# patrickzbhe/ray-tracing-series-rust

Hardware: AMD Instinct MI355X
Metric: Msamples/s (pixels x spp) on Book-1 final scene (higher is better)
Workload: dtype f64

## Files before the change

ray-tracing-series-rust_amd/csrc/hip/render.hip:

```cpp
#include <hip/hip_runtime.h>
#include <cstdio>
#include <cstdlib>
#include <algorithm>
#include <chrono>
#include <cfloat>
#include <cmath>
#include <cstring>
#include <new>
#include <type_traits>
#include <utility>
#include <string>
#include <vector>
#include "../../../include/rtx_abi.h"
#include "../core/cull32.hpp"
#include "../core/integrator.hpp"
#include "../core/occlusion.hpp"
#include "../core/item_order.hpp"
#include "../core/karras.hpp"
#include "../core/mover_box.hpp"
#include "../core/prim_box.hpp"
#include "../host/flat_scene.hpp"
#include "../host/light_table.hpp"
#include "../host/update_shadow.hpp"
#include "../host/set_shading.hpp"
#include "../host/wide_tree.hpp"
#include "device_buffer.hpp"
#include "f32_bridge.hpp"
#ifndef RTX_F32_TU
#include "abi_internal.hpp"
#include "../host/set_triangles.hpp"
#else
namespace rtx { void set_error(const std::string& msg); }
#endif

namespace rtx {

#include "lds_layout.inc"
#include "lds_variant.inc"
static_assert(LDSV_TIME_BOXES == RTX_LDS_VARIANT_TIME_BOXES && LDSV_ONE_AXIS == RTX_LDS_VARIANT_ONE_AXIS &&
              LDSV_COMMON_RATIO == RTX_LDS_VARIANT_COMMON_RATIO, "RtxRenderStats.trace_variant");
#include "pass_items.inc"

typedef const FlatNode4 FlatNode4Dev;
struct WorldDesc;

struct VoteTop {
  int32_t n;
  int32_t all_rects;
  int32_t k[8];
  uint32_t ref[8];
  rt::FlatRect rect[8];
};

enum class ForcedKernel { none, simple, vote, world, wavefront };

struct TraceSwitches {
  ForcedKernel kernel = ForcedKernel::none;
  bool diag = false;
  int ring = -1, wide = -1, scene_lds = -1;
  bool vote_top = true, tri_direct = true, mat_lds = true, perlin_lds = true;
  bool mv_common = true, motion = true, motion_axis = true;
  bool single_leaf = true, pass_pipeline = true, validate = false;
  uint32_t chunk = TRACE_CHUNK;
  uint32_t item_group = 0;
  uint32_t world_threshold = 8;
  uint32_t walk_threshold = 0, regen_min = 0, leaf_weight = 0;
  uint32_t wf_paths = 1u << 22, wf_refill = 16, wf_check = 8;
  int wf_occ = 4;
  bool wf_verbose = false;
};

struct Workspace {
  DeviceBuffer<double> samples;
  DeviceBuffer<double> accum;
  DeviceBuffer<rt::TraceCounters> counters;
  DeviceBuffer<unsigned int> work_counter;
  DeviceBuffer<PassMap> pass_map;
  DeviceBuffer<unsigned long long> diag;
  hipEvent_t ev[2] = {nullptr, nullptr};
  hipStream_t aux_stream = nullptr;
  hipEvent_t ev_pass[3] = {nullptr, nullptr, nullptr};
  DeviceBuffer<unsigned char> wave_mem;
  uint32_t* wave_host_ctrl = nullptr;
};

struct VotePlan {
  bool ok = false;
  int32_t bvh_pos = 0;
  int32_t tri_base = -1;
  VoteTop top;
  int blocks_per_cu[2] = {1, 1};
  bool ring[2] = {false, false};
  uint32_t tables = 0;
  size_t tables_bytes = 0;
};

struct WidePlan {
  FlatNode4Dev* nodes4 = nullptr;
  int levels = 0;
  int vote_blocks_per_cu = 1;
};

struct WorldPlan {
  const WorldDesc* desc = nullptr;
  uint32_t mat_lds = 0, tex_lds = 0;
  uint32_t perlin_lds = 0;
  int blocks_per_cu[5][2] = {{1, 1}, {1, 1}, {1, 1}, {1, 1}, {1, 1}};
};

struct LdsFit {
  bool ok = false;
  uint32_t ring_cap = 0;
  uint32_t levels = 0;
  LdsSceneDims dims = {0, 0, 0, 0, 0, 0};
};

struct LdsPlan {
  LdsFit plain;
  LdsFit motion;
  int motion_axis = -1;
  double motion_t0 = 0.0, motion_t1 = 0.0;
  bool motion_planned = false;
  uint32_t lds_max = 0;
  bool mv_common = false;
  double mv_t0 = 0.0, mv_t1 = 1.0;
};

struct WalkTuning {
  uint32_t walk_threshold = 18;
  uint32_t regen_min = 1;
  uint32_t leaf_weight = 3;
  bool single_leaf = false;
  uint32_t item_group_lds = 2, item_group_vote = rt::ITEM_GROUP_MAX, item_group_world = 4,
           item_group_wavefront = rt::ITEM_GROUP_MAX, item_group_simple = rt::ITEM_GROUP_MAX;
};

struct SceneUpdate {
  UpdateShadow shadow;
  std::vector<double> local_box;
  size_t n_entries = 0, n_nodes = 0, n_motion = 0, n_desc = 0;
  size_t n_triangles = 0, n_top = 0, n_spheres = 0, n_moving_spheres = 0, n_rects = 0;
  DeviceBuffer<double> d_local_box;
  DeviceBuffer<int32_t> d_leaf_parent, d_node_parent;
  DeviceBuffer<unsigned int> d_arrivals;
  DeviceBuffer<rt::XformOp64> d_slot_ops64;
  StagingBuffer staging;
  ShadingShadow shading;
  int32_t member_stack = 0;
  std::vector<int32_t> tree_depth;
  size_t n_perlins = 0, n_materials = 0, n_textures = 0;
  DeviceBuffer<double> r_boxes, r_bounds, r_box64, r_terms;
  DeviceBuffer<unsigned long long> r_keys, r_keys_sorted;
  DeviceBuffer<uint32_t> r_vals, r_vals_sorted;
  DeviceBuffer<int32_t> r_children, r_parent_node, r_parent_leaf, r_leaf_parent, r_node_parent, r_depth;
  DeviceBuffer<rt::FlatNode> r_nodes;
  DeviceBuffer<rt::FlatNode32> r_nodes32;
  DeviceBuffer<rt::FlatMotion32> r_motion32;
  DeviceBuffer<unsigned char> r_sort_temp;
};

#ifndef RTX_F32_TU
struct MeshUpdate {
  MeshShadow shadow;
  bool uploaded = false;
  DeviceBuffer<int32_t> d_leaves, d_node_parent;
  DeviceBuffer<unsigned int> d_arrivals;
  StagingBuffer staging;
  bool local_box_stale = false;
  std::vector<char> sphere_is_light;
  std::vector<char> rect_is_light;
  DeviceBuffer<double> d_light_weight;
  std::vector<unsigned int> slope_mask;
  DeviceBuffer<unsigned int> d_slope_mask;
  DeviceBuffer<double> d_end_boxes;
  ReadbackWords slope_readback;
};
#endif

struct DeviceScene {
  int device = -1;
  std::vector<DeviceBuffer<void>> allocations;
  rt::SceneView view;
  size_t scene_bytes = 0;
  int n_cu = 256;
  double gravity_time_limit = 1e300;
  TraceSwitches sw;
  Workspace ws;
  VotePlan vote;
  WidePlan wide;
  WorldPlan world;
  LdsPlan lds;
  WalkTuning walk;
  rt::LightView lights = {nullptr, nullptr, 0, 0};
  SceneUpdate upd;
#ifndef RTX_F32_TU
  MeshUpdate mesh;
#endif
};

#define HIP_TRY(expr)                                                                      \
  do {                                                                                     \
    hipError_t _e = (expr);                                                                \
    if (_e != hipSuccess) {                                                                \
      set_error(std::string(#expr) + ": " + hipGetErrorString(_e));                        \
      return RTX_EHIP;                                                                     \
    }                                                                                      \
  } while (0)

template <class T>
static rtx_status upload_array(DeviceScene* ds, const std::vector<T>& v, const T** out) {
  *out = nullptr;
  if (v.empty()) return RTX_OK;
  DeviceBuffer<void> b;
  size_t bytes = v.size() * sizeof(T);
  HIP_TRY(b.alloc(bytes));
// ... 61 lines not shown
#include "trace_vote.inc"
#include "trace_world.inc"
#include "trace_lds.inc"
#include "trace_wave.inc"
#include "post_kernels.inc"
#include "denoise.inc"
#include "cast_rays.inc"
#include "trace_rays.inc"
#include "occlusion.inc"
#ifndef RTX_F32_TU
#include "trace_nee.inc"
#endif
#include "scene_update.inc"
static size_t stack_bytes(uint32_t levels);
static void plan_world_stacks(DeviceScene* ds);
#include "scene_rebuild.inc"
#ifndef RTX_F32_TU
#include "mesh_update.inc"
#endif
#include "shading_update.inc"
#include "cull_hooks.inc"

static int shard_row_count(int32_t height, const RtxShard& sh, int32_t row_limit) {
  int n = 0;
  for (int32_t j = 0; j < height && j < row_limit; ++j)
    if ((j / sh.block_rows) % sh.shard_count == sh.shard_index) ++n;
  return n;
}

static rtx_status validate(const void* s, const RtxCamera* cam, const RtxConfig* cfg,
                           const RtxShard* shard, RtxShard* sh_out) {
  if (!s || !cam || !cfg) { set_error("render: NULL scene, camera or config"); return RTX_EINVAL; }
  if (cfg->threads <= 0 || cfg->image_width <= 0 || cfg->samples_per_pixel <= 0 || cfg->max_depth <= 0) {
    set_error("render: Config::new asserts threads, image_width, samples_per_pixel, max_depth > 0 (world.rs:36-40)");
    return RTX_EINVAL;
  }
  if (rtx_image_height(cfg) <= 0) { set_error("render: image height <= 0 (Screen::new asserts, screen.rs:14)"); return RTX_EINVAL; }
  if (!(cam->time1 < cam->time2)) { set_error("render: camera time1 >= time2 (gen_range panics on an empty range, camera.rs:69)"); return RTX_EINVAL; }
  RtxShard sh = {0, 1, 1, 0};
  if (shard) sh = *shard;
  if (sh.shard_count <= 0 || sh.shard_index < 0 || sh.shard_index >= sh.shard_count || sh.block_rows <= 0) {
    set_error("render: bad shard");
    return RTX_EINVAL;
  }
  *sh_out = sh;
  return RTX_OK;
}

static rt::RenderParams make_params(const RtxCamera* cam, const RtxConfig* cfg) {
  rt::RenderParams rp;
  static_assert(sizeof(RtxCamera) == 24 * sizeof(double) && sizeof(rt::FlatCamera) == 24 * sizeof(rt::real), "camera layout");
  for (int k = 0; k < 24; ++k) ((rt::real*)&rp.cam)[k] = (rt::real)((const double*)cam)[k];
  rp.background = rt::v3(cfg->background[0], cfg->background[1], cfg->background[2]);
  rp.image_width = cfg->image_width;
  rp.image_height = rtx_image_height(cfg);
  rp.samples_per_pixel = cfg->samples_per_pixel;
  rp.max_depth = cfg->max_depth;
  rp.seed = cfg->seed;
  return rp;
}

static TraceSwitches read_switches() {
  auto num = [](const char* n, int lo, int hi, uint32_t dflt) { const char* s = getenv(n); return s && atoi(s) >= lo && atoi(s) <= hi ? (uint32_t)atoi(s) : dflt; };
  auto flag = [](const char* n) { const char* s = getenv(n); return s ? (atoi(s) != 0 ? 1 : 0) : -1; };
  TraceSwitches sw;
  if (const char* k = getenv("RTX_TRACE_KERNEL")) {
    const std::string s = k;
    if (s == "simple") sw.kernel = ForcedKernel::simple;
    else if (s == "vote" || s == "vote_diag") sw.kernel = ForcedKernel::vote;
    else if (s == "world" || s == "world_diag") sw.kernel = ForcedKernel::world;
    else if (s == "wavefront") sw.kernel = ForcedKernel::wavefront;
    sw.diag = s == "vote_diag" || s == "world_diag";
  }
  sw.ring = flag("RTX_RING"); sw.wide = flag("RTX_WIDE"); sw.scene_lds = flag("RTX_SCENE_LDS");
  sw.vote_top = flag("RTX_VOTE_TOP") != 0; sw.tri_direct = flag("RTX_TRI_DIRECT") != 0;
  sw.mat_lds = flag("RTX_MAT_LDS") != 0; sw.perlin_lds = flag("RTX_PERLIN_LDS") != 0;
  sw.mv_common = flag("RTX_MV_COMMON") != 0; sw.motion = flag("RTX_MOTION") != 0; sw.motion_axis = flag("RTX_MOTION_AXIS") != 0;
  sw.single_leaf = flag("RTX_SINGLE_LEAF") != 0; sw.pass_pipeline = flag("RTX_PASS_PIPELINE") != 0;
  sw.validate = getenv("RTX_VALIDATE") != nullptr;
  sw.chunk = num("RTX_CHUNK", 64, 65536, sw.chunk);
  sw.item_group = num("RTX_ITEM_GROUP", 1, (int)rt::ITEM_GROUP_MAX, 0);
  sw.world_threshold = num("RTX_WORLD_THRESHOLD", 0, 64, sw.world_threshold);
  sw.walk_threshold = num("RTX_WALK_THRESHOLD", 1, 64, 0); sw.regen_min = num("RTX_REGEN_MIN", 1, 64, 0); sw.leaf_weight = num("RTX_LEAF_WEIGHT", 1, 64, 0);
  const char* wp = getenv("RTX_WF_PATHS");
  if (wp && atol(wp) >= 256 && atol(wp) <= (1l << 27)) sw.wf_paths = (uint32_t)atol(wp);
  sw.wf_refill = num("RTX_WF_REFILL", 1, 64, sw.wf_refill); sw.wf_check = num("RTX_WF_CHECK", 1, 4096, sw.wf_check);
  sw.wf_occ = (int)num("RTX_WF_OCC", 4, 6, (uint32_t)sw.wf_occ); sw.wf_verbose = getenv("RTX_WF_VERBOSE") != nullptr;
  return sw;
}

static size_t stack_bytes(uint32_t levels) { return (size_t)levels * TRACE_BLOCK * sizeof(int32_t); }

template <class K>
static int occupancy(K kernel, size_t lds) {
  int nb = 0;
  return hipOccupancyMaxActiveBlocksPerMultiprocessor(&nb, kernel, TRACE_BLOCK, lds) == hipSuccess ? nb : 0;
}

static uint32_t grid_size(uint32_t total, uint32_t block, uint64_t resident) {
  const uint64_t want = ((uint64_t)total + block - 1) / block;
  return (uint32_t)(want < resident ? want : resident);
}

struct PassArgs {
  rt::RenderParams rp;
  ShardMap sm;
  uint32_t s_begin, total, npix;
  double* samples;
  unsigned int* work_counter;
  hipStream_t stream;
  int preset;
  uint32_t feat;
  uint32_t stack_levels;
  size_t stack_lds;
  const uint32_t* active;
};

template <class Launch>
static void with_map(const PassArgs& a, Launch launch) {
  if (a.active) launch(ActiveMap{a.sm, a.active});
  else launch(a.sm);
}

template <class Launch>
static rtx_status run_diag(DeviceScene* ds, hipStream_t stream, Launch launch, const char* tag, int width, const char* const* names,
                           int n, unsigned long long (&h)[24]) {
  if (!ds->ws.diag) HIP_TRY(ds->ws.diag.alloc(sizeof(h)));
  HIP_TRY(hipMemsetAsync(ds->ws.diag, 0, sizeof(h), stream));
  launch();
  HIP_TRY(hipStreamSynchronize(stream));
  HIP_TRY(hipMemcpy(h, ds->ws.diag, sizeof(h), hipMemcpyDeviceToHost));
  for (int k = 0; k < n; ++k)
    fprintf(stderr, "[%s] %-*s executions %llu lanes %llu mean lanes %.2f\n", tag, width, names[k], h[2 * k], h[2 * k + 1],
            h[2 * k] ? (double)h[2 * k + 1] / (double)h[2 * k] : 0.0);
  return RTX_OK;
}

struct LeafScan { uint32_t max_count = 0, max_end = 0; };
static LeafScan scan_leaves(const FlatScene& fs) {
  LeafScan s;
  for (const rt::FlatNode& nd : fs.nodes)
    for (int ch = 0; ch < 2; ++ch)
      if (nd.child[ch] < 0) {
        s.max_count = std::max(s.max_count, rt::leaf_count(nd.child[ch]));
        s.max_end = std::max(s.max_end, rt::leaf_first(nd.child[ch]) + rt::leaf_count(nd.child[ch]));
      }
  return s;
}

static void plan_vote(DeviceScene* ds, const FlatScene& fs) {
  VotePlan& p = ds->vote;
  const TraceSwitches& sw = ds->sw;
  const size_t lds = stack_bytes((uint32_t)fs.max_stack + 1u), lds_ring = lds + (TRACE_BLOCK / 64) * ring_bytes(64);
  const bool ring_fits = lds_ring <= 64 * 1024;
  auto fit = [&](int preset, int nb0, int nb1, bool ring_by_default) {
    p.ring[preset] = ring_by_default && nb1 > 0 && nb1 >= nb0 && ring_fits;
    if (sw.ring >= 0 && nb1 > 0 && ring_fits) p.ring[preset] = sw.ring != 0;
    const int nb = p.ring[preset] ? nb1 : nb0;
    if (nb > 0) p.blocks_per_cu[preset] = nb;
  };
  fit(0, occupancy(k_trace_vote<P_SPHERES, false, false, false>, lds), occupancy(k_trace_vote<P_SPHERES, false, true, false>, lds_ring), true);
  fit(1, occupancy(k_trace_vote<P_MESH, false, false, false>, lds), occupancy(k_trace_vote<P_MESH, false, true, false>, lds_ring), false);

  memset(&p.top, 0, sizeof(p.top));
  p.top.n = -1;
  int n_bvh = 0, n_other = 0;
// ... 242 lines not shown
static void plan_lds_motion_axis(LdsPlan* p, const TraceSwitches& sw, uint32_t slope_mask) {
  const bool y_only = slope_mask == 2u && sw.motion_axis;
  p->motion_axis = y_only ? 1 : -1;
  p->motion.dims.node_dwords = y_only ? LDSK_MOTION1_NODE_DWORDS : LDSK_MOTION_NODE_DWORDS;
  p->motion.ok = false;
  p->motion.ring_cap = 0;
  if (p->motion_planned && p->plain.ok) fit_lds(&p->motion, sw.ring != 0, p->lds_max);
}

static rtx_status plan_lds(DeviceScene* ds, const FlatScene& fs, const LeafScan& leaves) {
  const bool single_bvh = fs.top_level.size() == 1 && fs.entries[fs.top_level[0]].kind == rt::ENTRY_BVH;
  if (!single_bvh || (fs.features & ~P_SPHERES) != 0 || fs.nodes32.size() > LDSK_MAX_NODES) return RTX_OK;
  LdsPlan& p = ds->lds;
  const TraceSwitches& sw = ds->sw;
  const uint32_t max_end = leaves.max_end, levels = (uint32_t)fs.max_stack + 1u;
  int lds_max = 0;
  (void)hipDeviceGetAttribute(&lds_max, hipDeviceAttributeMaxSharedMemoryPerBlock, ds->device);
  if (lds_max > (int)LDSK_LDS_MAX) lds_max = (int)LDSK_LDS_MAX;
  p.plain.levels = levels;
  p.plain.dims = {(uint32_t)fs.nodes32.size(), max_end, max_end, 0u, LDSK_NODE_DWORDS, 0u};
  p.mv_common = sw.mv_common && lds_common_interval(fs.moving_spheres.data(), fs.moving_spheres.size(), &p.mv_t0, &p.mv_t1);
  uint32_t counts[3];
  lds_record_counts(fs.features, P_STATIC_SPHERES, (uint32_t)fs.spheres.size(), max_end, counts);
  p.plain.dims.n_spheres = counts[0]; p.plain.dims.n_moving = counts[1]; p.plain.dims.n_uni = counts[2];
  p.motion.levels = levels;
  p.motion.dims = p.plain.dims;
  p.motion.dims.node_dwords = LDSK_MOTION_NODE_DWORDS;
  if (leaves.max_count <= 4 && max_end <= LDSK_MAX_SLOTS && sw.scene_lds != 0 && lds_max > 0) {
    const bool want_ring = sw.ring != 0;
    fit_lds(&p.plain, want_ring, (uint32_t)lds_max);
    const rt::FlatEntry& be = fs.entries[fs.top_level[0]];
    if (p.plain.ok && !fs.motion32.empty() && (fs.features & rt::F_MOVING_SPHERE) && lds_motion_interval_ok((double)be.f[0], (double)be.f[1]) && sw.motion) {
      p.motion_t0 = (double)be.f[0]; p.motion_t1 = (double)be.f[1];
      p.motion_planned = true;
      p.lds_max = (uint32_t)lds_max;
    }
  }
  plan_lds_motion_axis(&p, sw, rt::motion_slope_mask(fs.motion32.data(), fs.motion32.size()));
  if (p.plain.ok) {
    hipError_t ae = hipSuccess;
    bool static_lds = false;
    hipFuncAttributes fa;
#define LDS_ATTR1(K)                                                                                                   \
  if (ae == hipSuccess) ae = hipFuncSetAttribute((const void*)K, hipFuncAttributeMaxDynamicSharedMemorySize, lds_max); \
  if (ae == hipSuccess) ae = hipFuncGetAttributes(&fa, (const void*)K);                                                \
  if (ae == hipSuccess && fa.sharedSizeBytes != 0) static_lds = true
#define LDS_ATTR(FEAT, RINGF, MOTIONF) LDS_ATTR1((k_trace_lds<FEAT, RINGF, MOTIONF>)); LDS_ATTR1((k_trace_lds<FEAT, RINGF, MOTIONF, ActiveMap>))
    LDS_ATTR(P_SPHERES, true, 0u); LDS_ATTR(P_SPHERES, false, 0u); LDS_ATTR(P_STATIC_SPHERES, true, 0u); LDS_ATTR(P_STATIC_SPHERES, false, 0u);
    LDS_ATTR(P_SPHERES, true, 1u); LDS_ATTR(P_SPHERES, false, 1u); LDS_ATTR(P_SPHERES, true, 3u); LDS_ATTR(P_SPHERES, false, 3u);
#undef LDS_ATTR
#undef LDS_ATTR1
    if (ae != hipSuccess) { (void)hipGetLastError(); p.plain.ok = false; p.motion.ok = false; }
    if (static_lds) {
      fprintf(stderr, "[rtx] k_trace_lds has static LDS in front of its node array: not used\n");
      p.plain.ok = false; p.motion.ok = false;
    }
  }
  if (sw.scene_lds >= 0) {
    auto bytes = [](const LdsFit& f) { return f.ok ? ldsk_layout(f.levels, f.ring_cap, f.dims).total : 0u; };
    fprintf(stderr, "[rtx] RTX_SCENE_LDS: k_trace_lds %s (ring of %u, %u B of LDS); time-aware boxes %s (ring of %u, %u B)\n",
            p.plain.ok ? "on" : "off", p.plain.ring_cap, ldsk_layout(levels, p.plain.ring_cap, p.plain.dims).total,
            p.motion.ok ? "on" : "off", p.motion.ring_cap, bytes(p.motion));
  }
  return RTX_OK;
}

static rtx_status launch_lds(DeviceScene* ds, const PassArgs& a, const RtxCamera* cam, int32_t* variant) {
#ifndef RTX_F32_TU
  if (ds->mesh.slope_readback.pending()) {
    const unsigned int* words = nullptr;
    HIP_TRY(ds->mesh.slope_readback.wait(&words));
    plan_lds_motion_axis(&ds->lds, ds->sw, words[0]);
  }
#endif
  const LdsPlan& p = ds->lds;
  *variant = lds_trace_variant(p.motion.ok, p.motion_t0, p.motion_t1, (double)cam->time1, (double)cam->time2, p.motion_axis, p.mv_common);
  const bool motion = (*variant & LDSV_TIME_BOXES) != 0;
  const LdsFit& f = motion ? p.motion : p.plain;
  const bool ring = f.ring_cap != 0u;
  const rt::real m_t0 = (rt::real)p.motion_t0, m_inv = (rt::real)(1.0 / (p.motion_t1 - p.motion_t0));
  const LdsKernelLayout L = ldsk_layout(f.levels, f.ring_cap, f.dims);
  const uint32_t grid = grid_size(a.total, LDSK_BLOCK, (uint64_t)ds->n_cu);
  const WalkTuning& wk = ds->walk;
#define LAUNCH_LDS2(FEAT, RINGF, MOTIONF)                                                                               \
  with_map(a, [&](auto map) {                                                                                           \
    hipLaunchKernelGGL(HIP_KERNEL_NAME(k_trace_lds<FEAT, RINGF, MOTIONF, decltype(map)>), dim3(grid), dim3(LDSK_BLOCK), L.total, \
                       a.stream, ds->view, a.rp, map, a.s_begin, a.total, a.samples, a.work_counter, wk.leaf_weight, \
                       wk.walk_threshold | (wk.single_leaf ? 0x100u : 0u), ds->sw.chunk, f.ring_cap, f.levels, f.dims,  \
                       m_t0, m_inv, p.mv_common ? 1u : 0u, (rt::real)p.mv_t0, (rt::real)p.mv_t1);                        \
  })
#define LAUNCH_LDS(FEAT, MOTIONF) do { if (ring) { LAUNCH_LDS2(FEAT, true, MOTIONF); } else { LAUNCH_LDS2(FEAT, false, MOTIONF); } } while (0)
  if (!lds_records_are_moving(a.feat, P_STATIC_SPHERES)) { LAUNCH_LDS(P_STATIC_SPHERES, 0u); }
  else if (*variant & LDSV_ONE_AXIS) { LAUNCH_LDS(P_SPHERES, 3u); }
  else if (motion) { LAUNCH_LDS(P_SPHERES, 1u); }
  else { LAUNCH_LDS(P_SPHERES, 0u); }
#undef LAUNCH_LDS
#undef LAUNCH_LDS2
  return RTX_OK;
}

template <bool COUNT>
static void launch_simple(const DeviceScene* ds, const PassArgs& a) {
  const uint32_t grid = grid_size(a.total, TRACE_BLOCK, (uint64_t)ds->n_cu * 8);
#define LAUNCH_SIMPLE2(FEAT, MAP)                                                                                       \
  hipLaunchKernelGGL(HIP_KERNEL_NAME(k_trace_simple<FEAT, COUNT, decltype(MAP)>), dim3(grid), dim3(TRACE_BLOCK), a.stack_lds, \
                     a.stream, ds->view, a.rp, MAP, a.s_begin, a.total, a.samples, ds->ws.counters)
#define LAUNCH_SIMPLE(FEAT) with_map(a, [&](auto map) { LAUNCH_SIMPLE2(FEAT, map); })
  const bool inst = (a.feat & rt::F_INSTANCE) != 0;
  if constexpr (COUNT) {
    if (inst) { LAUNCH_SIMPLE2(P_INST, a.sm); } else { LAUNCH_SIMPLE2(P_ALL, a.sm); }
  } else {
    if (a.preset == 0) { LAUNCH_SIMPLE(P_SPHERES); }
    else if (a.preset == 1) { LAUNCH_SIMPLE(P_MESH); }
    else if (inst) { LAUNCH_SIMPLE(P_INST); }
    else { LAUNCH_SIMPLE(P_ALL); }
  }
#undef LAUNCH_SIMPLE
#undef LAUNCH_SIMPLE2
}

#ifndef RTX_F32_TU
static rtx_status launch_nee(const DeviceScene* ds, const PassArgs& a) {
  const int preset = (a.feat & rt::F_INSTANCE) ? 3 : ((a.feat & ~P_MESH_ROOM) == 0 ? 0 : ((a.feat & rt::F_GRAVITY_SPHERE) ? 2 : 1));
#define LAUNCH_NEE(FEAT, MAP)                                                                                                   \
  do {                                                                                                                          \
    const int nb = occupancy(k_trace_nee<FEAT, decltype(MAP)>, a.stack_lds);                                                    \
    const uint32_t grid = grid_size(a.total, TRACE_CHUNK, (uint64_t)ds->n_cu * (uint64_t)(nb > 0 ? nb : 1) * (TRACE_BLOCK / 64)); \
    hipLaunchKernelGGL(HIP_KERNEL_NAME(k_trace_nee<FEAT, decltype(MAP)>), dim3((grid + TRACE_BLOCK / 64 - 1) / (TRACE_BLOCK / 64)),     \
                       dim3(TRACE_BLOCK), a.stack_lds, a.stream, ds->view, ds->lights, a.rp, MAP, a.s_begin, a.total,     \
                       a.samples, a.work_counter);                                                                              \
  } while (0)
  with_map(a, [&](auto map) {
    if (preset == 0) LAUNCH_NEE(P_MESH_ROOM, map);
    else if (preset == 1) LAUNCH_NEE(P_ANY, map);
    else if (preset == 3) LAUNCH_NEE(P_INST, map);
    else LAUNCH_NEE(P_ALL, map);
  });
#undef LAUNCH_NEE
  return RTX_OK;
}
#endif

static rtx_status wave_pass(DeviceScene* ds, const PassArgs& a) {
  Workspace& ws = ds->ws;
  const hipStream_t stream = a.stream;
  uint32_t P = ds->sw.wf_paths;
  if ((uint64_t)P > (uint64_t)a.total) P = a.total;
  P = (P + WF_SEG - 1u) & ~(WF_SEG - 1u);
  const uint32_t n_seg = P / WF_SEG;
  const size_t R = sizeof(rt::real);
  const size_t bytes = 64 + (size_t)P * (16 + 7 * R + 3 * R + 3 * R + R + 4 + 4 + 4 + 4) + (size_t)n_seg * 8;
  HIP_TRY(ws.wave_mem.grow(bytes, stream));
  if (!ws.wave_host_ctrl) HIP_TRY(hipHostMalloc((void**)&ws.wave_host_ctrl, 4 * sizeof(uint32_t), hipHostMallocDefault));
  WavePool pool;
  {
    unsigned char* m = ws.wave_mem;
    pool.ctrl = (uint32_t*)m; m += 64;
    pool.rng = (unsigned long long*)m; m += (size_t)P * 16;
    pool.ray = (rt::real*)m; m += (size_t)P * 7 * R;
    pool.product = (rt::real*)m; m += (size_t)P * 3 * R;
    pool.output = (rt::real*)m; m += (size_t)P * 3 * R;
    pool.hit_t = (rt::real*)m; m += (size_t)P * R;
    pool.depth = (int32_t*)m; m += (size_t)P * 4;
    pool.g = (uint32_t*)m; m += (size_t)P * 4;
    pool.hit_ref = (uint32_t*)m; m += (size_t)P * 4;
    pool.free_list = (uint32_t*)m; m += (size_t)P * 4;
    pool.n_free = (uint32_t*)m; m += (size_t)n_seg * 4;
    pool.cursor = (uint32_t*)m; m += (size_t)n_seg * 4;
    pool.P = P;
  }
  const int preset = a.preset;
  const bool wide = preset == 1 && ds->wide.nodes4 != nullptr;
  const uint32_t levels = wide ? (uint32_t)ds->wide.levels : a.stack_levels;
  const size_t lds = stack_bytes(levels);
  if (lds > 64 * 1024) { set_error("render: BVH too deep for the LDS traversal stack"); return RTX_EUNSUPPORTED; }
  const bool room = (a.feat & ~P_MESH_ROOM) == 0;
  const int occ = ds->sw.wf_occ;
  const uint32_t leaf_weight = ds->walk.leaf_weight, refill = ds->sw.wf_refill, bvh_pos = (uint32_t)ds->vote.bvh_pos;
#define WF_CASES(X)                                                                                                          \
  if (preset == 0) { X(P_SPHERES, false, 4); }                                                                               \
  else if (!wide) { X(P_MESH, false, 4); }                                                                                   \
  else if (room && occ == 5) { X(P_MESH_ROOM, true, 5); }                                                                    \
  else if (room && occ == 6) { X(P_MESH_ROOM, true, 6); }                                                                    \
  else if (room) { X(P_MESH_ROOM, true, 4); }                                                                                \
  else { X(P_MESH, true, 4); }
  int nb = 0;
  hipError_t oe = hipSuccess;
#define WF_OCC(FEAT, WIDEF, MB) oe = hipOccupancyMaxActiveBlocksPerMultiprocessor(&nb, k_wf_trace<FEAT, WIDEF, MB>, TRACE_BLOCK, lds)
  WF_CASES(WF_OCC)
#undef WF_OCC
  if (oe != hipSuccess || nb <= 0) { (void)hipGetLastError(); nb = 1; }
  const uint32_t tgrid = grid_size(P, TRACE_BLOCK, (uint64_t)ds->n_cu * (uint64_t)nb);
  hipLaunchKernelGGL(k_wf_init, dim3((P + 255u) / 256u), dim3(256), 0, stream, pool);
  uint32_t check_every = ds->sw.wf_check;
  int it = 0;
  for (;; ++it) {
    with_map(a, [&](auto map) {
      hipLaunchKernelGGL(HIP_KERNEL_NAME(k_wf_generate<decltype(map)>), dim3(n_seg), dim3(WF_SEG), 0, stream, pool, a.rp, map,
                         a.s_begin, a.total);
    });
    if ((uint32_t)(it + 1) % check_every == 0u) {
      HIP_TRY(hipMemsetAsync(pool.ctrl, 0, 16, stream));
      hipLaunchKernelGGL(k_wf_count, dim3(256), dim3(256), 0, stream, pool);
      HIP_TRY(hipGetLastError());
      HIP_TRY(hipMemcpyAsync(ws.wave_host_ctrl, pool.ctrl, 4 * sizeof(uint32_t), hipMemcpyDeviceToHost, stream));
      HIP_TRY(hipStreamSynchronize(stream));
      if (ws.wave_host_ctrl[0] == 0u) break;
      if (ws.wave_host_ctrl[0] < P / 2u) check_every = 2;
      if (it > 100000000) { set_error("render: wavefront integrator did not converge"); return RTX_EHIP; }
    }
#define WF_LAUNCH(FEAT, WIDEF, MB)                                                                                           \
  do {                                                                                                                       \
    hipLaunchKernelGGL(HIP_KERNEL_NAME(k_wf_trace<FEAT, WIDEF, MB>), dim3(tgrid), dim3(TRACE_BLOCK), lds, stream, ds->view, pool, \
                       leaf_weight, refill, bvh_pos, ds->wide.nodes4, ds->vote.tri_base);                                    \
    hipLaunchKernelGGL(HIP_KERNEL_NAME(k_wf_shade<FEAT>), dim3(n_seg), dim3(WF_SEG), 0, stream, ds->view, pool, a.rp, a.samples, bvh_pos); \
  } while (0)
    WF_CASES(WF_LAUNCH)
#undef WF_LAUNCH
  }
#undef WF_CASES
  if (ds->sw.wf_verbose) fprintf(stderr, "[rtx] wavefront: %u slots, %d iterations, %d blocks per CU (%u stack levels)\n", P, it + 1, nb, levels);
  return RTX_OK;
}

static void plan_walk(DeviceScene* ds, const LeafScan& leaves) {
  WalkTuning& w = ds->walk;
  const TraceSwitches& sw = ds->sw;
  w.leaf_weight = leaves.max_count <= 1 ? 1u : 3u;
  w.single_leaf = leaves.max_count <= 1;
  if (ds->wide.nodes4) { w.leaf_weight = 1u; w.walk_threshold = 24u; w.regen_min = 8u; }
  else if (ds->lds.plain.ok) w.walk_threshold = 12u;
  if (sw.regen_min) w.regen_min = sw.regen_min;
  if (sw.leaf_weight) w.leaf_weight = sw.leaf_weight;
  if (!sw.single_leaf) w.single_leaf = false;
  if (sw.walk_threshold) w.walk_threshold = sw.walk_threshold;
  if (sw.item_group) w.item_group_lds = w.item_group_vote = w.item_group_world = w.item_group_wavefront = w.item_group_simple = sw.item_group;
}

static uint32_t item_group_of(const WalkTuning& w, int32_t kernel) {
  switch (kernel) {
    case RTX_KERNEL_SIMPLE: return w.item_group_simple;
    case RTX_KERNEL_LDS: return w.item_group_lds;
    case RTX_KERNEL_WAVEFRONT: return w.item_group_wavefront;
    case RTX_KERNEL_VOTE: return w.item_group_vote;
    default: return w.item_group_world;
  }
}

static int32_t choose_trace_kernel(const DeviceScene* ds, int preset, bool count) {
  const ForcedKernel k = ds->sw.kernel;
  if (count || k == ForcedKernel::simple) return RTX_KERNEL_SIMPLE;
  if (ds->lds.plain.ok && preset == 0 && k == ForcedKernel::none) return RTX_KERNEL_LDS;
  if (ds->vote.ok && preset < 2 && k == ForcedKernel::wavefront) return RTX_KERNEL_WAVEFRONT;
  if (ds->vote.ok && preset < 2 && k != ForcedKernel::world) return RTX_KERNEL_VOTE;
  return RTX_KERNEL_WORLD;
}

typedef RtxSampleRange SampleRange;

struct PassPlan {
  uint32_t spp_pass;
  bool pipeline;
  size_t sample_bytes;
};

static rtx_status prepare_workspace(DeviceScene* ds, uint64_t sample_buffer_bytes, uint64_t npix, uint64_t npix_all, uint32_t spp,
                                    bool serial, hipStream_t stream, double** accum, PassPlan* pp) {
  Workspace& ws = ds->ws;
  uint64_t budget = sample_buffer_bytes;
  if (budget == 0) {
    budget = 24ull << 30;
    size_t free_b = 0, total_b = 0;
    if (hipMemGetInfo(&free_b, &total_b) == hipSuccess) {
      const uint64_t avail = ((uint64_t)free_b + ws.samples.bytes()) / 3;
      if (avail < budget) budget = avail;
    } else {
      (void)hipGetLastError();
    }
    if (budget < ws.samples.bytes()) budget = ws.samples.bytes();
  }
  const uint64_t per_sample_plane = npix * 24ull;
  uint32_t spp_pass = spp;
  const bool pipeline = ds->sw.pass_pipeline && !serial && ds->sw.kernel != ForcedKernel::simple && per_sample_plane > 0 &&
                        (uint64_t)spp * per_sample_plane > budget && budget / 2 >= per_sample_plane;
  const uint64_t pass_budget = pipeline ? budget / 2 : budget;
  if (per_sample_plane > 0 && (uint64_t)spp_pass * per_sample_plane > pass_budget) {
    spp_pass = (uint32_t)(pass_budget / per_sample_plane);
    if (spp_pass < 1) spp_pass = 1;
  }
  while (spp_pass > 1 && (uint64_t)spp_pass * npix >= 0xFFFF0000ull) --spp_pass;
  if ((uint64_t)spp_pass * npix >= 0xFFFF0000ull) { set_error("render: shard too large for one pass"); return RTX_EINVAL; }
  size_t need_samples = (size_t)spp_pass * per_sample_plane * (pipeline ? 2 : 1);
  if (need_samples > ws.samples.bytes()) {
    if (ws.samples) { HIP_TRY(hipStreamSynchronize(stream)); HIP_TRY(ws.samples.release()); }
    for (;;) {
      hipError_t me = ws.samples.alloc(need_samples);
      if (me == hipSuccess) break;
      (void)hipGetLastError();
      if (me != hipErrorOutOfMemory || spp_pass <= 1) {
        set_error(std::string("render: sample buffer of ") + std::to_string(need_samples) + " bytes: " + hipGetErrorString(me));
        return me == hipErrorOutOfMemory ? RTX_ENOMEM : RTX_EHIP;
      }
      spp_pass = (spp_pass + 1) / 2;
      need_samples = (size_t)spp_pass * per_sample_plane * (pipeline ? 2 : 1);
    }
  }
  if (!*accum) {
    HIP_TRY(ws.accum.grow((size_t)npix_all * 24, stream));
    *accum = ws.accum;
  }
  if (!ws.counters) HIP_TRY(ws.counters.alloc(sizeof(rt::TraceCounters)));
  if (!ws.work_counter) HIP_TRY(ws.work_counter.alloc(2 * sizeof(unsigned int)));
  if (!ws.pass_map) HIP_TRY(ws.pass_map.alloc(2 * sizeof(PassMap)));
  if (pipeline && !ws.aux_stream) {
    HIP_TRY(hipStreamCreateWithFlags(&ws.aux_stream, hipStreamNonBlocking));
    for (int i = 0; i < 3; ++i) HIP_TRY(hipEventCreateWithFlags(&ws.ev_pass[i], hipEventDisableTiming));
  }
  if (!ws.ev[0]) { HIP_TRY(hipEventCreate(&ws.ev[0])); HIP_TRY(hipEventCreate(&ws.ev[1])); }
// ... 893 lines not shown
```

ray-tracing-series-rust_amd/csrc/hip/trace_lds.inc:

```

#define LDSK_NO_REF 0xFFFFFFFFu
#ifndef LDSK_NODE_BURST
#define LDSK_NODE_BURST 1
#endif

typedef __attribute__((address_space(3))) unsigned char LdsByte;
typedef __attribute__((address_space(3))) float LdsF32;
typedef __attribute__((address_space(3))) int32_t LdsI32;
typedef __attribute__((address_space(3))) short LdsI16;
typedef __attribute__((address_space(3))) unsigned short LdsU16;
__device__ __forceinline__ const LdsByte* lds_at(uint32_t addr) { return (const LdsByte*)(uintptr_t)addr; }
struct LdsStack16 {
  uint32_t bottom, sp;
  __device__ __forceinline__ void init() { *(LdsU16*)lds_at(bottom) = 0xFFFFu; sp = bottom; }
  __device__ __forceinline__ void reset_with(uint32_t under) {
    sp = bottom + (under != 0xFFFFu ? LDSK_LEVEL_BYTES : 0u);
    set_top((int32_t)under);
  }
  __device__ __forceinline__ void set_top(int32_t v) { *(LdsU16*)lds_at(sp) = (unsigned short)v; }
  __device__ __forceinline__ void push(int32_t v) { sp += LDSK_LEVEL_BYTES; set_top(v); }
  __device__ __forceinline__ int32_t top() const { return (int32_t)*(const LdsI16*)lds_at(sp); }
  __device__ __forceinline__ int32_t pop() { const int32_t v = top(); sp -= LDSK_LEVEL_BYTES; return v; }
  __device__ __forceinline__ void move(bool hf, bool hs) {
    int32_t d = -1;
    d += (int32_t)hf;
    d += (int32_t)hs;
    sp += (uint32_t)d * LDSK_LEVEL_BYTES;
  }
};

template <uint32_t F, bool RING, uint32_t MOTION, class SM = ShardMap>
__global__ __launch_bounds__(LDSK_BLOCK) void k_trace_lds(rt::SceneView sv, rt::RenderParams rp, SM sm,
                                                          uint32_t s_begin, uint32_t total,
                                                          double* __restrict__ samples, unsigned int* work_counter,
                                                          uint32_t leaf_weight, uint32_t walk_threshold, uint32_t chunk, uint32_t ring_cap,
                                                          uint32_t stack_levels, LdsSceneDims dims, rt::real motion_t0, rt::real motion_inv_dt,
                                                          uint32_t mv_common, rt::real mv_t0, rt::real mv_t1) {
  static_assert(!MOTION || (F & rt::F_MOVING_SPHERE), "time-aware boxes only make sense with moving spheres");
  const bool single_leaf = (walk_threshold & 0x100u) != 0u;
  walk_threshold &= 0xFFu;
  constexpr bool UNI = (F & rt::F_MOVING_SPHERE) != 0;
  constexpr uint32_t FL = UNI ? (F & ~rt::F_SPHERE) : F;
  static_assert(MOTION <= 4u, "0: no slopes, 1: all axes, 2 + a: axis a only");
  constexpr uint32_t ND = MOTION == 1u ? LDSK_MOTION_NODE_DWORDS : (MOTION >= 2u ? LDSK_MOTION1_NODE_DWORDS : LDSK_NODE_DWORDS);
  constexpr uint32_t CBD = MOTION == 1u ? 19u : (MOTION >= 2u ? 13u : 10u);
  constexpr uint32_t MA = MOTION >= 2u ? MOTION - 2u : 0u;
  constexpr uint32_t CB = CBD * 4u;
  constexpr uint32_t ITEM_OFF = CB - 4u;
  constexpr uint32_t ROOT_ITEM_DWORD = 2u * CBD;
  static_assert((F & ~(rt::F_SPHERE | rt::F_MOVING_SPHERE | rt::F_BVH | rt::F_LAMBERTIAN | rt::F_METAL |
                       rt::F_DIELECTRIC | rt::F_CHECKER)) == 0, "k_trace_lds caches spheres and moving spheres only");
  extern __shared__ __attribute__((aligned(16))) unsigned char ldsk[];
  const LdsKernelLayout L = ldsk_layout(stack_levels, RING ? ring_cap : 0u, dims);
  const uint32_t lane = threadIdx.x & 63u;
  const rt::FlatEntry& bvh = sv.entries[sv.top_level[0]];
  int32_t entry_pair[2];
  lds_entry_pair(sv.nodes32, bvh.a, entry_pair);
  const uint32_t entry = ((uint32_t)entry_pair[0] & 0xFFFFu) | ((uint32_t)entry_pair[1] << 16);
  const uint32_t first_ref = (uint32_t)bvh.b;

  uint32_t* const lds_nodes = (uint32_t*)(ldsk + LDSK_OFF_NODES);
  rt::FlatSphere* const lds_spheres = (rt::FlatSphere*)(ldsk + L.off_spheres);
  rt::FlatMovingSphere* const lds_moving = (rt::FlatMovingSphere*)(ldsk + L.off_moving);
  {
    static_assert(sizeof(rt::FlatNode32) == 64 && offsetof(rt::FlatNode32, child) == 48 && offsetof(rt::FlatNode32, axis) == 56,
                  "the padded LDS copy assumes FlatNode32's layout");
    const uint32_t* src = (const uint32_t*)sv.nodes32;
    const uint32_t* msrc = (const uint32_t*)sv.motion32;
    for (uint32_t k = threadIdx.x; k < dims.n_nodes * 2u * CBD; k += LDSK_BLOCK) {
      const uint32_t node = k / (2u * CBD), field = k - node * (2u * CBD);
      const uint32_t c = field / CBD, r = field - c * CBD;
      uint32_t v;
      if (r < 9u) {
        const uint32_t a = r / 3u, t = r - a * 3u;
        v = MOTION ? msrc[node * 24u + (t == 1u ? 6u : 0u) + c * 3u + a]
                   : src[node * 16u + (t == 1u ? 6u : 0u) + c * 3u + a];
      } else if (MOTION == 1u && r < 18u) {
        const uint32_t a = (r - 9u) / 3u, t = (r - 9u) - a * 3u;
        v = msrc[node * 24u + (t == 1u ? 18u : 12u) + c * 3u + a];
      } else if (MOTION >= 2u && r < 12u) {
        const uint32_t t = r - 9u;
        v = msrc[node * 24u + (t == 1u ? 18u : 12u) + c * 3u + MA];
      } else {
        const int32_t child = (int32_t)src[node * 16u + 12u + c];
        int32_t item = ldsk_item(child);
        if (child >= 0) item |= sv.nodes32[child].axis << 13;
        v = (uint32_t)item;
      }
      lds_nodes[node * ND + field] = v;
    }
    if (threadIdx.x == 0) lds_nodes[ROOT_ITEM_DWORD] = (uint32_t)(bvh.a | (sv.nodes32[bvh.a].axis << 13));
    if (UNI) {
      for (uint32_t k = threadIdx.x; k < dims.n_refs; k += LDSK_BLOCK) {
        const rt::PrimRef ref = sv.refs[first_ref + k];
        rt::FlatMovingSphere m;
        if (rt::primref_type(ref) == rt::PRIM_SPHERE) {
          const rt::FlatSphere sp = sv.spheres[rt::primref_index(ref)];
          m.c0[0] = sp.cx; m.c0[1] = sp.cy; m.c0[2] = sp.cz; m.c1[0] = sp.cx; m.c1[1] = sp.cy; m.c1[2] = sp.cz;
          m.time0 = rt::real(0.0); m.time1 = rt::real(1.0); m.radius = sp.radius; m.mat = sp.mat; m.pad = 0;
        } else {
          m = sv.moving_spheres[rt::primref_index(ref)];
        }
        lds_moving[k] = m;
      }
    } else {
      constexpr uint32_t SD = (uint32_t)(sizeof(rt::FlatSphere) / 4);
      uint32_t* ds = (uint32_t*)lds_spheres;
      const uint32_t* ss = (const uint32_t*)sv.spheres;
      for (uint32_t k = threadIdx.x; k < dims.n_refs * SD; k += LDSK_BLOCK) {
        const uint32_t slot = k / SD, field = k - slot * SD;
        ds[k] = ss[rt::primref_index(sv.refs[first_ref + slot]) * SD + field];
      }
    }
  }
  __syncthreads();
  rt::SceneView lsv = sv;
  lsv.spheres = lds_spheres;
  lsv.moving_spheres = lds_moving;

  LdsStack16 stack;
  stack.bottom = (uint32_t)(uintptr_t)(LdsByte*)ldsk + L.off_stacks + threadIdx.x * 2u;
  stack.init();
  double* const ring_f = (double*)(ldsk + L.off_ring + (threadIdx.x >> 6) * ring_bytes(ring_cap));
  uint32_t* const ring_g = (uint32_t*)(ring_f + RING_F64 * ring_cap);
  uint32_t ring_n = 0;
  uint32_t chunk_pos = 0, chunk_end = 0;
  bool queue_empty = false;
  bool active = false;
  uint32_t g = 0;
  rt::PathState ps;
  bool midwalk = false;
  rt::Ray32 q = {0.f, 0.f, 0.f, 0.f, 0.f, 0.f, 0.f, 0.f};
  uint32_t dir_neg = 0;
  uint32_t off_x = 0, off_y = 12, off_z = 24;
  uint32_t flip_b = 0;
  float t_max32 = 0.f;
  float s32 = 0.f;
  rt::real mv_ratio = rt::real(0.0);
  int32_t cur = LDSK_DONE;
  rt::Closest best;
  best.t = 0.0; best.ref = LDSK_NO_REF; best.order = 0; best.hit = false;

  for (;;) {
    const unsigned long long need_mask = wave_ballot(!active);
    if (need_mask != 0ull) {
      const uint32_t n_need = (uint32_t)__popcll(need_mask);
      const uint32_t rank = lane_rank(need_mask);
      if (RING) {
#define RING_CAP ring_cap
#define RING_DIAG(mask)
#include "trace_ring.inc"
#undef RING_DIAG
#undef RING_CAP
      } else {
        if (chunk_pos >= chunk_end && !queue_empty) {
          uint32_t base = 0;
          if (lane == 0) base = atomicAdd(work_counter, chunk);
          base = __builtin_amdgcn_readfirstlane(base);
          if (base >= total) {
            queue_empty = true;
          } else {
            chunk_pos = base;
            chunk_end = (total - base < chunk) ? total : base + chunk;
          }
        }
        if (chunk_pos < chunk_end) {
          const uint32_t avail = chunk_end - chunk_pos;
          if (!active && rank < avail) {
            g = start_path(rp, sm, s_begin, chunk_pos + rank, &ps);
            active = true;
          }
          chunk_pos += (n_need < avail) ? n_need : avail;
        }
      }
    }
    if (wave_ballot(active) == 0ull) break;
    if (active && !midwalk) {
      if (rt::path_bounce_begin(&ps)) {
        store_sample(samples, g, ps.output);
        active = false;
      } else {
        q = rt::make_ray32(ps.ray, rt::ray_t_min(ps.ray));
        dir_neg = rt::ray32_dir_neg(q);
        off_x = (dir_neg & 1u) << 2; off_y = 12u + ((dir_neg & 2u) << 1); off_z = 24u + (dir_neg & 4u);
        flip_b = ((dir_neg & 1u) * CB) | (((dir_neg >> 1) & 1u) * (CB << 8)) | (((dir_neg >> 2) & 1u) * (CB << 16));
        t_max32 = __builtin_huge_valf();
        if (UNI && mv_common != 0u) mv_ratio = (ps.ray.time - mv_t0) / (mv_t1 - mv_t0);
        if (MOTION) s32 = __builtin_fminf(__builtin_fmaxf((float)((ps.ray.time - motion_t0) * motion_inv_dt), 0.f), 1.f);
        best.t = RT_INFINITY; best.ref = LDSK_NO_REF; best.order = 0;
        uint32_t e = entry;
        asm volatile("" : "+s"(e));
        cur = (int32_t)(short)e;
        stack.reset_with(e >> 16);
        float fin = (q.oix + q.oiy) + q.oiz;
        if (UNI) fin += (float)ps.ray.time;
        if (!__builtin_amdgcn_classf(__builtin_fmaf(fin, 0.f, (q.ix * q.iy) * q.iz), 0x198u)) {
          cur = *(const LdsI32*)lds_at(LDSK_OFF_NODES + ROOT_ITEM_DWORD * 4u);
          stack.sp = stack.bottom;
        }
        midwalk = true;
      }
    }
    const uint32_t threshold = (queue_empty && ring_n == 0u) ? 1u : walk_threshold;
    auto node_step = [&]() {
      const LdsByte* nd = lds_at(LDSK_OFF_NODES + ((uint32_t)cur & 0x1FFFu) * (ND * 4u));
      const uint32_t first_b = __builtin_amdgcn_ubfe(flip_b, ((uint32_t)cur >> 10) & 0x18u, 8u);
      const LdsByte* bf = nd + first_b;
      const LdsByte* bs = nd + (CB - first_b);
      const LdsF32 *fx = (const LdsF32*)(bf + off_x), *fy = (const LdsF32*)(bf + off_y), *fz = (const LdsF32*)(bf + off_z);
      const LdsF32 *sx = (const LdsF32*)(bs + off_x), *sy = (const LdsF32*)(bs + off_y), *sz = (const LdsF32*)(bs + off_z);
      int32_t top = stack.top();
      bool hf, hs;
      if (MOTION >= 2u) {
        constexpr uint32_t SO = 9u - 3u * MA;
        const auto* fm = MA == 0u ? fx : (MA == 1u ? fy : fz);
        const auto* sm = MA == 0u ? sx : (MA == 1u ? sy : sz);
        const float fn = __builtin_fmaf(s32, fm[SO], fm[0]), ff = __builtin_fmaf(s32, fm[SO + 1u], fm[1]);
        const float sn = __builtin_fmaf(s32, sm[SO], sm[0]), sf = __builtin_fmaf(s32, sm[SO + 1u], sm[1]);
        hf = rt::cull32_may_hit_nf_pos(MA == 0u ? fn : fx[0], MA == 0u ? ff : fx[1], MA == 1u ? fn : fy[0], MA == 1u ? ff : fy[1],
                                       MA == 2u ? fn : fz[0], MA == 2u ? ff : fz[1], q, t_max32);
        hs = rt::cull32_may_hit_nf_pos(MA == 0u ? sn : sx[0], MA == 0u ? sf : sx[1], MA == 1u ? sn : sy[0], MA == 1u ? sf : sy[1],
                                       MA == 2u ? sn : sz[0], MA == 2u ? sf : sz[1], q, t_max32);
      } else if (MOTION) {
        hf = rt::cull32_may_hit_nf_pos(__builtin_fmaf(s32, fx[9], fx[0]), __builtin_fmaf(s32, fx[10], fx[1]), __builtin_fmaf(s32, fy[9], fy[0]),
                                   __builtin_fmaf(s32, fy[10], fy[1]), __builtin_fmaf(s32, fz[9], fz[0]), __builtin_fmaf(s32, fz[10], fz[1]), q, t_max32);
        hs = rt::cull32_may_hit_nf_pos(__builtin_fmaf(s32, sx[9], sx[0]), __builtin_fmaf(s32, sx[10], sx[1]), __builtin_fmaf(s32, sy[9], sy[0]),
                                   __builtin_fmaf(s32, sy[10], sy[1]), __builtin_fmaf(s32, sz[9], sz[0]), __builtin_fmaf(s32, sz[10], sz[1]), q, t_max32);
      } else {
        hf = rt::cull32_may_hit_nf_pos(fx[0], fx[1], fy[0], fy[1], fz[0], fz[1], q, t_max32);
        hs = rt::cull32_may_hit_nf_pos(sx[0], sx[1], sy[0], sy[1], sz[0], sz[1], q, t_max32);
      }
      int32_t cf = *(const LdsI32*)(bf + ITEM_OFF), cs = *(const LdsI32*)(bs + ITEM_OFF);
      asm volatile("" : "+v"(top), "+v"(cf), "+v"(cs));
      const bool both = hf && hs;
      cur = hf ? cf : (hs ? cs : top);
      stack.move(hf, hs);
      if (both) stack.set_top(cs);
    };
    auto leaf_test = [&](uint32_t slot) {
      const rt::PrimRef ref = rt::make_primref(UNI ? rt::PRIM_MOVING_SPHERE : rt::PRIM_SPHERE, slot);
      rt::real t;
      bool ok;
      if (UNI && mv_common != 0u) {
        const rt::FlatMovingSphere& sp = lds_moving[slot];
        const rt::Point3 c0 = rt::load_v3(sp.c0), c1 = rt::load_v3(sp.c1);
        ok = rt::sphere_root(c0 + mv_ratio * (c1 - c0), sp.radius, ps.ray, rt::ray_t_min(ps.ray), best.t, &t);
      } else {
        ok = rt::prim_t<FL, false>(lsv, ref, ps.ray, rt::ray_t_min(ps.ray), best.t, &t, nullptr);
      }
      if (ok && !(t == best.t && slot < best.order)) { best.t = t; best.ref = ref; best.order = slot; }
    };
    {
      bool is_node = cur >= 0;
      bool is_leaf = cur < -1;
      uint32_t n_node = (uint32_t)__popcll(wave_ballot(is_node)), n_leaf = (uint32_t)__popcll(wave_ballot(is_leaf));
      if (n_node + n_leaf >= threshold) {
        do {
          if (n_node * leaf_weight >= n_leaf) {
            if (is_node) node_step();
#if LDSK_NODE_BURST >= 2
            if (cur >= 0) node_step();
#endif
          } else {
            if (is_leaf) {
              const uint32_t f = ((uint32_t)cur & 0x7FFFu) >> 2;
              if (single_leaf) {
                leaf_test(f);
              } else {
                const uint32_t k = ((uint32_t)cur & 3u) + 1u;
                for (uint32_t i = 0; i < k; ++i) leaf_test(f + i);
              }
              t_max32 = rt::cull_round_up(best.t);
              cur = stack.pop();
            }
          }
          is_node = cur >= 0;
          is_leaf = cur < -1;
          n_node = (uint32_t)__popcll(wave_ballot(is_node));
          n_leaf = (uint32_t)__popcll(wave_ballot(is_leaf));
        } while (n_node + n_leaf >= threshold);
      }
    }
    if (midwalk && cur == LDSK_DONE) {
      midwalk = false;
      rt::HitRecord rec;
      const bool hit = best.ref != LDSK_NO_REF;
      if (hit) rt::prim_finalize<FL>(lsv, best.ref, ps.ray, best.t, &rec);
      if (rt::path_bounce_end<F, false>(sv, rp, &ps, hit, rec, nullptr)) {
        store_sample(samples, g, ps.output);
        active = false;
      }
    }
  }
}
```

Before: 8713.

## Add early retire rounds in ring LDS traversal to shade missed rays in batches

In the ring variant of the LDS trace kernel, the walk loop can now exit early once a set number of lanes (retire_done) have finished. Finished lanes whose rays missed are then shaded or retired only if enough of them are done together (retire_min). The walk threshold for the ring path drops to a separate lower default. The aim is to cut divergence idle time by letting finished lanes refill sooner, at the cost of more loop iterations and extra ballot overhead.

```diff
diff --git a/ray-tracing-series-rust_amd/csrc/hip/render.hip b/ray-tracing-series-rust_amd/csrc/hip/render.hip
--- a/ray-tracing-series-rust_amd/csrc/hip/render.hip
+++ b/ray-tracing-series-rust_amd/csrc/hip/render.hip
@@ -54,6 +54,7 @@
 
 enum class ForcedKernel { none, simple, vote, world, wavefront };
 
+constexpr uint32_t RETIRE_UNSET = 0xFFFFFFFFu;
 struct TraceSwitches {
   ForcedKernel kernel = ForcedKernel::none;
   bool diag = false;
@@ -65,6 +66,7 @@
   uint32_t item_group = 0;
   uint32_t world_threshold = 8;
   uint32_t walk_threshold = 0, regen_min = 0, leaf_weight = 0;
+  uint32_t retire_done = RETIRE_UNSET, retire_min = RETIRE_UNSET;
   uint32_t wf_paths = 1u << 22, wf_refill = 16, wf_check = 8;
   int wf_occ = 4;
   bool wf_verbose = false;
@@ -131,6 +133,7 @@
   uint32_t regen_min = 1;
   uint32_t leaf_weight = 3;
   bool single_leaf = false;
+  uint32_t retire_done = 44, retire_min = 18, retire_walk_threshold = 10;
   uint32_t item_group_lds = 2, item_group_vote = rt::ITEM_GROUP_MAX, item_group_world = 4,
            item_group_wavefront = rt::ITEM_GROUP_MAX, item_group_simple = rt::ITEM_GROUP_MAX;
 };
@@ -358,6 +361,7 @@
   sw.item_group = num("RTX_ITEM_GROUP", 1, (int)rt::ITEM_GROUP_MAX, 0);
   sw.world_threshold = num("RTX_WORLD_THRESHOLD", 0, 64, sw.world_threshold);
   sw.walk_threshold = num("RTX_WALK_THRESHOLD", 1, 64, 0); sw.regen_min = num("RTX_REGEN_MIN", 1, 64, 0); sw.leaf_weight = num("RTX_LEAF_WEIGHT", 1, 64, 0);
+  sw.retire_done = num("RTX_RETIRE_DONE", 0, 64, RETIRE_UNSET); sw.retire_min = num("RTX_RETIRE_MIN", 0, 64, RETIRE_UNSET);
   const char* wp = getenv("RTX_WF_PATHS");
   if (wp && atol(wp) >= 256 && atol(wp) <= (1l << 27)) sw.wf_paths = (uint32_t)atol(wp);
   sw.wf_refill = num("RTX_WF_REFILL", 1, 64, sw.wf_refill); sw.wf_check = num("RTX_WF_CHECK", 1, 4096, sw.wf_check);
@@ -766,11 +770,13 @@
   const LdsKernelLayout L = ldsk_layout(f.levels, f.ring_cap, f.dims);
   const uint32_t grid = grid_size(a.total, LDSK_BLOCK, (uint64_t)ds->n_cu);
   const WalkTuning& wk = ds->walk;
+  const uint32_t tuning = ((ring && wk.retire_done) ? wk.retire_walk_threshold : wk.walk_threshold) | (wk.single_leaf ? 0x100u : 0u) |
+                          ((wk.retire_done ? wk.retire_done : 127u) << 16) | (wk.retire_min << 24);
 #define LAUNCH_LDS2(FEAT, RINGF, MOTIONF)                                                                               \
   with_map(a, [&](auto map) {                                                                                           \
     hipLaunchKernelGGL(HIP_KERNEL_NAME(k_trace_lds<FEAT, RINGF, MOTIONF, decltype(map)>), dim3(grid), dim3(LDSK_BLOCK), L.total, \
                        a.stream, ds->view, a.rp, map, a.s_begin, a.total, a.samples, a.work_counter, wk.leaf_weight, \
-                       wk.walk_threshold | (wk.single_leaf ? 0x100u : 0u), ds->sw.chunk, f.ring_cap, f.levels, f.dims,  \
+                       tuning, ds->sw.chunk, f.ring_cap, f.levels, f.dims,  \
                        m_t0, m_inv, p.mv_common ? 1u : 0u, (rt::real)p.mv_t0, (rt::real)p.mv_t1);                        \
   })
 #define LAUNCH_LDS(FEAT, MOTIONF) do { if (ring) { LAUNCH_LDS2(FEAT, true, MOTIONF); } else { LAUNCH_LDS2(FEAT, false, MOTIONF); } } while (0)
@@ -917,7 +923,9 @@
   if (sw.regen_min) w.regen_min = sw.regen_min;
   if (sw.leaf_weight) w.leaf_weight = sw.leaf_weight;
   if (!sw.single_leaf) w.single_leaf = false;
-  if (sw.walk_threshold) w.walk_threshold = sw.walk_threshold;
+  if (sw.walk_threshold) w.walk_threshold = w.retire_walk_threshold = sw.walk_threshold;
+  if (sw.retire_done != RETIRE_UNSET) w.retire_done = sw.retire_done;
+  if (sw.retire_min != RETIRE_UNSET) w.retire_min = sw.retire_min;
   if (sw.item_group) w.item_group_lds = w.item_group_vote = w.item_group_world = w.item_group_wavefront = w.item_group_simple = sw.item_group;
 }
 
diff --git a/ray-tracing-series-rust_amd/csrc/hip/trace_lds.inc b/ray-tracing-series-rust_amd/csrc/hip/trace_lds.inc
--- a/ray-tracing-series-rust_amd/csrc/hip/trace_lds.inc
+++ b/ray-tracing-series-rust_amd/csrc/hip/trace_lds.inc
@@ -38,7 +38,8 @@
                                                           uint32_t mv_common, rt::real mv_t0, rt::real mv_t1) {
   static_assert(!MOTION || (F & rt::F_MOVING_SPHERE), "time-aware boxes only make sense with moving spheres");
   const bool single_leaf = (walk_threshold & 0x100u) != 0u;
-  walk_threshold &= 0xFFu;
+  const uint32_t tuning = walk_threshold;
+  if (!RING) walk_threshold &= 0xFFu;
   constexpr bool UNI = (F & rt::F_MOVING_SPHERE) != 0;
   constexpr uint32_t FL = UNI ? (F & ~rt::F_SPHERE) : F;
   static_assert(MOTION <= 4u, "0: no slopes, 1: all axes, 2 + a: axis a only");
@@ -201,7 +202,10 @@
         midwalk = true;
       }
     }
-    const uint32_t threshold = (queue_empty && ring_n == 0u) ? 1u : walk_threshold;
+    const bool no_refill = queue_empty && ring_n == 0u;
+    uint32_t tn = tuning;
+    if (RING) asm volatile("" : "+s"(tn));
+    const uint32_t threshold = no_refill ? 1u : (RING ? (tn & 0xFFu) : walk_threshold);
     auto node_step = [&]() {
       const LdsByte* nd = lds_at(LDSK_OFF_NODES + ((uint32_t)cur & 0x1FFFu) * (ND * 4u));
       const uint32_t first_b = __builtin_amdgcn_ubfe(flip_b, ((uint32_t)cur >> 10) & 0x18u, 8u);
@@ -250,11 +254,14 @@
       }
       if (ok && !(t == best.t && slot < best.order)) { best.t = t; best.ref = ref; best.order = slot; }
     };
+    bool round_over = true;
     {
       bool is_node = cur >= 0;
       bool is_leaf = cur < -1;
       uint32_t n_node = (uint32_t)__popcll(wave_ballot(is_node)), n_leaf = (uint32_t)__popcll(wave_ballot(is_leaf));
-      if (n_node + n_leaf >= threshold) {
+      int32_t exit_at = (int32_t)threshold;
+      if (RING) exit_at = max(exit_at, (int32_t)(n_node + n_leaf) - (int32_t)(no_refill ? 127u : ((tn >> 16) & 0x7Fu)));
+      if (n_node + n_leaf >= (uint32_t)exit_at) {
         do {
           if (n_node * leaf_weight >= n_leaf) {
             if (is_node) node_step();
@@ -278,10 +285,18 @@
           is_leaf = cur < -1;
           n_node = (uint32_t)__popcll(wave_ballot(is_node));
           n_leaf = (uint32_t)__popcll(wave_ballot(is_leaf));
-        } while (n_node + n_leaf >= threshold);
-      }
-    }
-    if (midwalk && cur == LDSK_DONE) {
+        } while (n_node + n_leaf >= (uint32_t)exit_at);
+      }
+      if (RING) round_over = n_node + n_leaf < threshold;
+    }
+    bool shade = midwalk && cur == LDSK_DONE;
+    if (!round_over) {
+      shade = shade && best.ref == LDSK_NO_REF;
+      uint32_t tm = tuning;
+      asm volatile("" : "+s"(tm));
+      if ((uint32_t)__popcll(wave_ballot(shade)) < (tm >> 24)) shade = false;
+    }
+    if (shade) {
       midwalk = false;
       rt::HitRecord rec;
       const bool hit = best.ref != LDSK_NO_REF;
```

After: 8854, median of 6. 1.02x the previous value.
